# APRIL-ZJU/Ctrl-VIO

Hardware: NVIDIA H100
Metric: residual+Jacobian block evaluations per second (sliding-window LM solve) (higher is better)
Workload: dtype f64

## Files before the change

### ctrl-vio_b200/csrc/engine.cu

```cuda
#include <atomic>
#include <cmath>
#include <cstdlib>
#include <map>

#include "engine_state.h"
#include "poly_min.h"

namespace {

int refresh_mirror(ctvio_engine* e, cudaStream_t on = nullptr) {
  const size_t need = 4 * size_t(e->nK) + kPStride * size_t(e->nK) + 6 * size_t(std::max(e->nB, 1)) + size_t(std::max(e->nL, 1)) + 8;
  if (need > e->h_mirror_cap) {
    if (e->h_mirror) cudaFreeHost(e->h_mirror);
    e->h_mirror = nullptr;
    e->h_mirror_cap = 0;
    if (cudaHostAlloc(reinterpret_cast<void**>(&e->h_mirror), (2 * need) * sizeof(double), cudaHostAllocDefault) != cudaSuccess) {
      cudaGetLastError();
      e->mirror_valid = false;
      return CTVIO_OK;
    }
    e->h_mirror_cap = 2 * need;
  }
  DevState& x = e->x[e->cur];
  double* m = e->h_mirror;
// ... 53 lines not shown
      if (c.t != t) { c.t = t; c.ok = knot_window(e, t, c.f, c.l); }
      f = c.f; l = c.l;
      return c.ok;
    };
    for (int k = 0; k < n; ++k) {
      const HostImage& o = e->img[k];
      int f0, l0, f1, l1;
      if (!window_of(o.ti, f0, l0) || !window_of(o.tj, f1, l1))
        return fail(CTVIO_ERR_TIME_RANGE, "image factor time (+ rolling-shutter padding) outside the spline");
      if (o.lm < 0 || o.lm >= e->nL) return fail(CTVIO_ERR_INVALID, "landmark index out of range");
      wi0[k] = f0; wj0[k] = f1;
      e->img_li[k] = l0; e->img_lj[k] = l1;
      e->h_lo[o.lm] = std::min(e->h_lo[o.lm], 6 * std::min(f0, f1));
      e->h_hi[o.lm] = std::max(e->h_hi[o.lm], 6 * (std::max(l0, l1) + 1));
    }
    e->img_order.resize(n);
    {
      bool lm_sorted = true;
      for (int k = 1; k < n && lm_sorted; ++k) lm_sorted = e->img[k - 1].lm <= e->img[k].lm;
      const size_t nKk = size_t(e->nK) + 1;
      if (lm_sorted && nKk * nKk <= (size_t(1) << 22)) {
        std::vector<int32_t> start(nKk * nKk + 1, 0);
        for (int k = 0; k < n; ++k) ++start[size_t(wi0[k]) * nKk + size_t(wj0[k]) + 1];
        for (size_t g = 1; g < start.size(); ++g) start[g] += start[g - 1];
        for (int k = 0; k < n; ++k) e->img_order[start[size_t(wi0[k]) * nKk + size_t(wj0[k])]++] = k;
      } else {
        std::vector<uint64_t> key(n);
        const uint64_t nLl = uint64_t(std::max(e->nL, 1));
        if (uint64_t(nKk) * nKk * nLl < (uint64_t(1) << 40) && uint64_t(n) < (uint64_t(1) << 24)) {
          for (int k = 0; k < n; ++k)
            key[k] = (((uint64_t(wi0[k]) * nKk + uint64_t(wj0[k])) * nLl + uint64_t(e->img[k].lm)) << 24) | uint64_t(k);
          std::sort(key.begin(), key.end());
          for (int k = 0; k < n; ++k) e->img_order[k] = int32_t(key[k] & 0xffffffu);
        } else {
          for (int k = 0; k < n; ++k) e->img_order[k] = k;
          std::stable_sort(e->img_order.begin(), e->img_order.end(), [&](int a, int b) {
            if (wi0[a] != wi0[b]) return wi0[a] < wi0[b];
            if (wj0[a] != wj0[b]) return wj0[a] < wj0[b];
            return e->img[a].lm < e->img[b].lm;
          });
        }
      }
    }
    std::vector<longlong2> ht(n);
    std::vector<double2> hpi(n), hpj(n);
    std::vector<int4> hm(n);
    for (int k = 0; k < n; ++k) {
      const HostImage& o = e->img[e->img_order[k]];
      ht[k] = make_longlong2(o.ti, o.tj);
      hpi[k] = make_double2(o.pi[0], o.pi[1]);
      hpj[k] = make_double2(o.pj[0], o.pj[1]);
      hm[k] = make_int4(o.rowi, o.rowj, o.lm, o.marg);
    }
    constexpr int cap = kVisObsPerRound;
    std::vector<VisualItem>& items = e->h_items;
    items.clear();
    for (int k = 0; k < n;) {
      const int a = e->img_order[k];
      int end = k;
      while (end < n && wi0[e->img_order[end]] == wi0[a] && wj0[e->img_order[end]] == wj0[a]) ++end;
      const int cnt = end - k;
      const int nchunks = (cnt + cap - 1) / cap;
      const int per = (cnt + nchunks - 1) / nchunks;
      for (int s = k; s < end; s += per) items.push_back(VisualItem{s, std::min(per, end - s), wi0[a], wj0[a]});
      k = end;
    }
    e->n_items = int(items.size());
    if (!e->img_desc.empty()) {
      std::vector<ctvio::FactorDesc> sd(n);
      for (int k = 0; k < n; ++k) sd[k] = e->img_desc[e->img_order[k]];
      CUDA_OK(e->d_img_desc.upload(sd, st));
      CUDA_OK(e->d_img_t.reserve(n)); CUDA_OK(e->d_img_pi.reserve(n)); CUDA_OK(e->d_img_pj.reserve(n)); CUDA_OK(e->d_img_meta.reserve(n));
      ctvio::GatherFactorsArgs ga;
      ga.n = n; ga.desc = e->d_img_desc.p; ga.table = e->d_frames.p; ga.frame_t = e->d_frame_t.p;
      ga.frame_cap = ctvio_engine::kFrameCap;
      ga.t = e->d_img_t.p; ga.pi = e->d_img_pi.p; ga.pj = e->d_img_pj.p; ga.meta = e->d_img_meta.p;
      e->launches += ctvio::launch_gather_factors(ga, st);
    } else {
      CUDA_OK(e->d_img_t.upload(ht, st));
      CUDA_OK(e->d_img_pi.upload(hpi, st));
      CUDA_OK(e->d_img_pj.upload(hpj, st));
      CUDA_OK(e->d_img_meta.upload(hm, st));
    }
    CUDA_OK(e->d_img_orig.upload(e->img_order, st));
    CUDA_OK(e->d_items.upload(items, st));

    e->h_woff.assign(e->nL + 1, 0);
    for (int l = 0; l < e->nL; ++l) {
      if (e->h_hi[l] == 0) e->h_lo[l] = 0;
      e->h_woff[l + 1] = e->h_woff[l] + (e->h_hi[l] - e->h_lo[l]);
    }
    CUDA_OK(e->d_lo.upload(e->h_lo, st));
    CUDA_OK(e->d_hi.upload(e->h_hi, st));
    CUDA_OK(e->d_woff.upload(e->h_woff, st));
    const int ni = int(e->imu.size());
    std::vector<longlong2> it(ni);
    std::vector<double2> iga(3 * size_t(ni));
    const int64_t maxt = e->cfg.t0_ns + int64_t(e->nK - 3) * e->cfg.dt_ns;
    std::vector<int32_t>& imu_order = e->imu_order;
    imu_order.assign(ni, 0);
    std::vector<int32_t> imu_s(ni);
    for (int k = 0; k < ni; ++k) {
      const HostImu& o = e->imu[k];
      if (o.t < e->cfg.t0_ns || o.t >= maxt) return fail(CTVIO_ERR_TIME_RANGE, "imu time outside the spline");
      if (o.node < 0 || o.node >= e->nB) return fail(CTVIO_ERR_INVALID, "bias node out of range");
      imu_order[k] = k;
      imu_s[k] = knot_window_first(e, o.t);
    }
    std::stable_sort(imu_order.begin(), imu_order.end(), [&](int a, int b) {
      if (imu_s[a] != imu_s[b]) return imu_s[a] < imu_s[b];
      return e->imu[a].node < e->imu[b].node;
    });
    std::vector<ImuItem> imu_items;
    for (int k = 0; k < ni; ++k) {
      const HostImu& o = e->imu[imu_order[k]];
      it[k] = make_longlong2(o.t, o.node);
      iga[3 * k] = make_double2(o.gyro[0], o.gyro[1]);
      iga[3 * k + 1] = make_double2(o.gyro[2], o.accel[0]);
// ... 1727 lines not shown
```

### ctrl-vio_b200/csrc/kernels.h

```cpp
#pragma once
#include <cuda_runtime.h>

#include <atomic>

#include <cstdint>
#include <utility>

#include "spline_eval.cuh"

namespace ctvio {

constexpr int kPStride = 4;
constexpr int kVisThreads = 256;
constexpr int kVisObsPerRound = 128;
constexpr int kLocalDim = 64;
constexpr int kRowStride = 66;
constexpr int kObsStride = 2 * kRowStride + 2;
constexpr int kWinKnots = 5;
constexpr int kColLd = 60, kColR = 61, kColRho = 62;
constexpr int kCholNB = 64;

struct StatePtrs {
  double* q;
  double* p;
  double* bias;
  double* rho;
  double* ld;
  KnotPair* tab;
};

struct NormalEqPtrs {
  double* A;
  double* gc;
  double* hl;
  double* gl;
  double* wld;
  double* W;
  double* cost;
};

struct ImageObsPtrs {
  const longlong2* t;
  const double2* pi;
  const double2* pj;
  const int4* meta;
  int32_t n;
};

struct VisualItem {
  int32_t start, count;
  int32_t wi0, wj0;
};

struct ImuObsPtrs {
  const longlong2* t_node;
  const double2* ga;
  int32_t n;
};

struct ImuItem {
  int32_t start, count;
  int32_t s, node;
};
constexpr int kImuMaxPerItem = 32;

struct BiasFactorPtrs {
  const int2* ij;
// ... 263 lines not shown
```

### ctrl-vio_b200/csrc/kernels_residual.cu

```cuda
#include <cstdio>

#include "kernels.h"

namespace ctvio {


__device__ __forceinline__ uint32_t smem_u32(const void* p) { return static_cast<uint32_t>(__cvta_generic_to_shared(p)); }

__device__ __forceinline__ void mbar_init(uint64_t* bar, uint32_t count) {
  asm volatile("mbarrier.init.shared::cta.b64 [%0], %1;" ::"r"(smem_u32(bar)), "r"(count) : "memory");
}
__device__ __forceinline__ void fence_mbar_init() { asm volatile("fence.mbarrier_init.release.cluster;" ::: "memory"); }
__device__ __forceinline__ void mbar_expect_tx(uint64_t* bar, uint32_t bytes) {
  asm volatile("mbarrier.arrive.expect_tx.shared::cta.b64 _, [%0], %1;" ::"r"(smem_u32(bar)), "r"(bytes) : "memory");
}
__device__ __forceinline__ void tma_bulk_g2s(void* dst, const void* src, uint32_t bytes, uint64_t* bar) {
  asm volatile("cp.async.bulk.shared::cluster.global.mbarrier::complete_tx::bytes [%0], [%1], %2, [%3];" ::"r"(
                   smem_u32(dst)),
               "l"(src), "r"(bytes), "r"(smem_u32(bar))
               : "memory");
}
__device__ __forceinline__ bool mbar_try_wait(uint64_t* bar, uint32_t phase) {
  uint32_t ok;
  asm volatile(
// ... 11 lines not shown
__device__ __forceinline__ double warp_sum(double v) {
#pragma unroll
  for (int o = 16; o > 0; o >>= 1) v += __shfl_xor_sync(0xffffffffu, v, o);
  return v;
}


__global__ void knot_table_kernel(StatePtrs st, int nK) {
  const int k = blockIdx.x * blockDim.x + threadIdx.x;
  if (k >= nK - 1) return;
  KnotPair kp;
  make_knot_pair(st.q, k, kp);
  st.tab[k] = kp;
}

int launch_knot_table(const StatePtrs& st, int nK, cudaStream_t s) {
  if (nK < 2) return 0;
  knot_table_kernel<<<(nK - 1 + 127) / 128, 128, 0, s>>>(st, nK);
  return 1;
}


struct VisArgs {
  ImageObsPtrs obs;
  const VisualItem* items;
  StatePtrs st;
  NormalEqPtrs ne;
  LandmarkLayout lm;
  ProblemDims dims;
  SplineParams sp;
  RigParams rig;
  double cauchy;
  const uint8_t* cmask;
  LmScalars* scal;
  int* det_ticket;
};

struct __align__(128) VisStatic {
  KnotPair tab[2][4];
  double q[2][kWinKnots][4];
  double p[2][kWinKnots][4];
  double cost_part[8];
  unsigned long long bar;
  int err;
};

__constant__ uint8_t c_tile_i[36] = {0, 0, 0, 0, 0, 0, 0, 0, 1, 1, 1, 1, 1, 1, 1, 2, 2, 2,
                                     2, 2, 2, 3, 3, 3, 3, 3, 4, 4, 4, 4, 5, 5, 5, 6, 6, 7};
__constant__ uint8_t c_tile_j[36] = {0, 1, 2, 3, 4, 5, 6, 7, 1, 2, 3, 4, 5, 6, 7, 2, 3, 4,
                                     5, 6, 7, 3, 4, 5, 6, 7, 4, 5, 6, 7, 5, 6, 7, 6, 7, 7};

#ifdef CTVIO_CHOL_TIMING
__device__ long long g_vis_clk[8];
#define VCLK(i) do { if (blockIdx.x == 0 && threadIdx.x == 0) g_vis_clk[(i)] = clock64(); } while (0)
extern "C" int ctvio_debug_vis_clk(long long* out) {
  return cudaMemcpyFromSymbol(out, g_vis_clk, sizeof(g_vis_clk)) == cudaSuccess ? 0 : -1;
}
#else
#define VCLK(i)
#endif

size_t visual_smem_bytes() {
  return size_t(kVisObsPerRound) * kObsStride * sizeof(double) + size_t(36) * 64 * sizeof(double);
}

__device__ __noinline__ void syrk_round(const double* Jt, double* accs, int nround, int tid) {
  const int warp = tid >> 5, lane = tid & 31, g = lane >> 2, q = lane & 3;
  const int nblk = warp < 6 ? 1 : 2;
  int bi[2], bj[2];
  if (warp < 6) {
    bi[0] = warp < 3 ? 0 : (warp < 5 ? 1 : 2);
    bj[0] = warp < 3 ? warp + 1 : (warp < 5 ? warp - 1 : 3);
    bi[1] = bj[1] = 0;
  } else {
    bi[0] = bj[0] = 2 * (warp - 6);
    bi[1] = bj[1] = 2 * (warp - 6) + 1;
  }
  const bool dg = warp >= 6;
  double acc[2][2][2][2];
#pragma unroll
  for (int b = 0; b < 2; ++b)
#pragma unroll
    for (int mi = 0; mi < 2; ++mi)
#pragma unroll
      for (int nj = 0; nj < 2; ++nj) {
        const int ti = 2 * bi[b] + mi, tj = 2 * bj[b] + nj;
        double2 v = make_double2(0.0, 0.0);
        if (b < nblk && ti <= tj) v = *reinterpret_cast<const double2*>(accs + (ti * 8 - ti * (ti - 1) / 2 + (tj - ti)) * 64 + g * 8 + 2 * q);
        acc[b][mi][nj][0] = v.x; acc[b][mi][nj][1] = v.y;
      }
  const int nsteps = (2 * nround + 3) >> 2;
#pragma unroll 2
  for (int st = 0; st < nsteps; ++st) {
    const int row = 4 * st + q;
    const double* rp = Jt + size_t(row >> 1) * kObsStride + (row & 1) * kRowStride + g;
#pragma unroll
    for (int b = 0; b < 2; ++b) {
      if (b < nblk) {
        double av[2], bv[2];
#pragma unroll
        for (int m = 0; m < 2; ++m) {
          av[m] = rp[16 * bi[b] + 8 * m];
          bv[m] = dg ? av[m] : rp[16 * bj[b] + 8 * m];
        }
#pragma unroll
        for (int mi = 0; mi < 2; ++mi)
#pragma unroll
          for (int nj = 0; nj < 2; ++nj) {
            if (dg && mi == 1 && nj == 0) continue;
            asm volatile("mma.sync.aligned.m8n8k4.row.col.f64.f64.f64.f64 {%0,%1}, {%2}, {%3}, {%0,%1};"
                         : "+d"(acc[b][mi][nj][0]), "+d"(acc[b][mi][nj][1])
                         : "d"(av[mi]), "d"(bv[nj]));
          }
      }
    }
  }
#pragma unroll
  for (int b = 0; b < 2; ++b)
#pragma unroll
    for (int mi = 0; mi < 2; ++mi)
#pragma unroll
      for (int nj = 0; nj < 2; ++nj) {
        const int ti = 2 * bi[b] + mi, tj = 2 * bj[b] + nj;
        if (b < nblk && ti <= tj)
          *reinterpret_cast<double2*>(accs + (ti * 8 - ti * (ti - 1) / 2 + (tj - ti)) * 64 + g * 8 + 2 * q) =
              make_double2(acc[b][mi][nj][0], acc[b][mi][nj][1]);
      }
  __syncthreads();
}

template <bool FULL>
__global__ void __launch_bounds__(kVisThreads, 1) visual_kernel(const __grid_constant__ VisArgs a) {
  extern __shared__ __align__(128) unsigned char dyn_smem[];
  double* Jt = reinterpret_cast<double*>(dyn_smem);
  double* accs = Jt + size_t(kVisObsPerRound) * kObsStride;
  __shared__ VisStatic sm;

  const int tid = threadIdx.x;
  const int lane = tid & 31, warp = tid >> 5;
  const VisualItem item = a.items[blockIdx.x];
  const int nK = a.dims.nK;
  VCLK(0);

  const int w0[2] = {item.wi0, item.wj0};
  if (tid == 0) {
    sm.err = 0;
    mbar_init(reinterpret_cast<uint64_t*>(&sm.bar), 1);
    fence_mbar_init();
  }
  __syncthreads();
  if (tid == 0) {
    uint32_t bytes = 0;
#pragma unroll
    for (int sd = 0; sd < 2; ++sd) {
      const int nk = min(kWinKnots, nK - w0[sd]);
      const int npair = min(4, nK - 1 - w0[sd]);
      bytes += uint32_t(nk) * 64u + uint32_t(npair) * uint32_t(sizeof(KnotPair));
    }
    mbar_expect_tx(reinterpret_cast<uint64_t*>(&sm.bar), bytes);
#pragma unroll
    for (int sd = 0; sd < 2; ++sd) {
      const int nk = min(kWinKnots, nK - w0[sd]);
      const int npair = min(4, nK - 1 - w0[sd]);
      tma_bulk_g2s(&sm.q[sd][0][0], a.st.q + 4 * w0[sd], uint32_t(nk) * 32u, reinterpret_cast<uint64_t*>(&sm.bar));
      tma_bulk_g2s(&sm.p[sd][0][0], a.st.p + 4 * w0[sd], uint32_t(nk) * 32u, reinterpret_cast<uint64_t*>(&sm.bar));
      tma_bulk_g2s(&sm.tab[sd][0], a.st.tab + w0[sd], uint32_t(npair) * uint32_t(sizeof(KnotPair)),
                   reinterpret_cast<uint64_t*>(&sm.bar));
    }
  }
  if (FULL)
    for (int i = tid; i < 36 * 64; i += kVisThreads) accs[i] = 0.0;
  while (!mbar_try_wait(reinterpret_cast<uint64_t*>(&sm.bar), 0)) {
  }
  __syncthreads();

  const double ld = *a.st.ld;
  const int64_t ld_ns = int64_t(ld * 1e9);
  const int side = tid & 1;
  double cost_local = 0.0;
  VCLK(1);
// ... 180 lines not shown
        const int gb = sb == 0 ? 6 * item.wi0 + lb : (sb == 1 ? 6 * item.wj0 + (lb - 30) : a.dims.idx_ld);
        if (n_class > 1) {
          int c;
          if (sb == 2) c = 5 + sa;
          else if (sa == sb) c = sa == 0 ? 0 : 4;
          else c = ga < gb ? 1 : (ga > gb ? 2 : 3);
          if (c != cls) continue;
        }
        const double v = (la != lb && ga == gb) ? 2.0 * val : val;
        const int g0 = min(ga, gb), g1 = max(ga, gb);
        atomicAdd(a.ne.A + size_t(g0) * np + g1, v);
      }
      if (n_class > 1) {
        __threadfence();
        __syncthreads();
      }
    }
  }
  if (a.det_ticket) {
    __threadfence();
    __syncthreads();
    if (tid == 0) asm volatile("st.release.gpu.global.s32 [%0], %1;" ::"l"(a.det_ticket), "r"((int(blockIdx.x) + 1) * 1024) : "memory");
  }
  VCLK(5);
}

int launch_visual(const VisualLaunch& l, bool full, cudaStream_t s) {
  if (l.n_items <= 0) return 0;
  VisArgs a{l.obs, l.items, l.st, l.ne, l.lm, l.dims, l.sp, l.rig, l.cauchy, l.cmask, l.scal, l.det_ticket};
  static PerDeviceOnce once;
  if (once.first()) {
    cudaFuncSetAttribute(visual_kernel<true>, cudaFuncAttributeMaxDynamicSharedMemorySize, int(visual_smem_bytes()));
    cudaFuncSetAttribute(visual_kernel<false>, cudaFuncAttributeMaxDynamicSharedMemorySize, int(visual_smem_bytes()));
  }
  if (full) visual_kernel<true><<<l.n_items, kVisThreads, visual_smem_bytes(), s>>>(a);
  else visual_kernel<false><<<l.n_items, kVisThreads, 0, s>>>(a);
  return 1;
}


struct ImuArgs {
  ImuObsPtrs obs;
  const ImuItem* items;
  StatePtrs st;
  NormalEqPtrs ne;
  ProblemDims dims;
  SplineParams sp;
  RigParams rig;
  const uint8_t* cmask;
  LmScalars* scal;
  int* det_ticket;
};

constexpr int kImuThreads = 64;
constexpr int kImuCols = 32;
constexpr int kImuRowStride = 34;
__constant__ uint8_t c_imu_tile_i[10] = {0, 0, 0, 0, 1, 1, 1, 2, 2, 3};
__constant__ uint8_t c_imu_tile_j[10] = {0, 1, 2, 3, 1, 2, 3, 2, 3, 3};

template <bool FULL>
__global__ void __launch_bounds__(kImuThreads) imu_kernel(const __grid_constant__ ImuArgs a) {
  extern __shared__ __align__(16) unsigned char dyn_smem[];
  double* Js = reinterpret_cast<double*>(dyn_smem);
  double* accs = Js + kImuMaxPerItem * 6 * kImuRowStride;
  const int tid = threadIdx.x;
  const ImuItem item = a.items[blockIdx.x];
  double cost = 0.0;
  if (FULL)
    for (int i = tid; i < 10 * 64; i += kImuThreads) accs[i] = 0.0;
  if (tid < item.count) {
    const int n = item.start + tid;
    const longlong2 tn = a.obs.t_node[n];
    const double2 g0 = a.obs.ga[3 * n], g1 = a.obs.ga[3 * n + 1], g2 = a.obs.ga[3 * n + 2];
    const double gyro[3] = {g0.x, g0.y, g1.x}, accel[3] = {g1.y, g2.x, g2.y};
    const int node = item.node;
    double bias[6];
#pragma unroll
    for (int c = 0; c < 6; ++c) bias[c] = a.st.bias[6 * node + c];
    int32_t s;
    double u;
    const bool ok = spline_index(a.sp, tn.x, s, u) && s == item.s;
    double* J = Js + size_t(tid) * 6 * kImuRowStride;
    if (!ok) {
      atomicOr(&a.scal->error_flags, 1);
      if (FULL)
        for (int e = 0; e < 6 * kImuRowStride; ++e) J[e] = 0.0;
    } else {
      ImuEvalOut o;
      eval_imu<FULL, kPStride>(a.sp, a.rig, a.st.q, a.st.p, a.st.tab, s, u, gyro, accel, bias, o);
      cost = o.cost;
      if (FULL) {
        const int gb0 = a.dims.idx_bias0 + 6 * node;
#pragma unroll
        for (int r = 0; r < 6; ++r) {
          double* Jr = J + r * kImuRowStride;
#pragma unroll
          for (int k = 0; k < 4; ++k)
#pragma unroll
            for (int c = 0; c < 3; ++c) {
              Jr[k * 6 + c] = a.cmask[6 * (s + k) + c] ? 0.0 : o.Jrot[k][3 * r + c];
              Jr[k * 6 + 3 + c] = a.cmask[6 * (s + k) + 3 + c] ? 0.0 : o.Jpos[k][3 * r + c];
            }
#pragma unroll
          for (int c = 0; c < 6; ++c) Jr[24 + c] = (c == r && !a.cmask[gb0 + c]) ? a.rig.imu_info[r] : 0.0;
          Jr[30] = o.r[r];
          Jr[31] = 0.0;
        }
      }
    }
  }
  if (FULL) {
    __syncthreads();
    const int grp = tid / 10, tile = tid % 10;
    double acc[64];
    if (tid < 60) {
      const int ti = c_imu_tile_i[tile], tj = c_imu_tile_j[tile];
#pragma unroll
      for (int e = 0; e < 64; ++e) acc[e] = 0.0;
      const int nrows = 6 * item.count;
      for (int row = grp; row < nrows; row += 6) {
        const double2* ra = reinterpret_cast<const double2*>(Js + size_t(row) * kImuRowStride + ti * 8);
        const double2* rb = reinterpret_cast<const double2*>(Js + size_t(row) * kImuRowStride + tj * 8);
        double av[8], bv[8];
#pragma unroll
        for (int e = 0; e < 4; ++e) {
          const double2 x = ra[e], y = rb[e];
          av[2 * e] = x.x; av[2 * e + 1] = x.y;
          bv[2 * e] = y.x; bv[2 * e + 1] = y.y;
        }
#pragma unroll
        for (int i = 0; i < 8; ++i)
#pragma unroll
          for (int j = 0; j < 8; ++j) acc[i * 8 + j] = fma(av[i], bv[j], acc[i * 8 + j]);
      }
    }
    for (int g = 0; g < 6; ++g) {
      if (tid < 60 && grp == g) {
#pragma unroll
        for (int e = 0; e < 64; ++e) accs[tile * 64 + e] += acc[e];
      }
      __syncthreads();
    }
    const int np = a.dims.np;
    det_ticket_wait(a.det_ticket, blockIdx.x);
    for (int idx = tid; idx < 10 * 64; idx += kImuThreads) {
      const double val = accs[idx];
      if (val == 0.0) continue;
      const int tile2 = idx >> 6, e = idx & 63;
      const int la = c_imu_tile_i[tile2] * 8 + (e >> 3), lb = c_imu_tile_j[tile2] * 8 + (e & 7);
      if (la > lb || lb > 30 || la >= 30) continue;
      const int ga = la < 24 ? 6 * item.s + la : a.dims.idx_bias0 + 6 * item.node + (la - 24);
      if (lb == 30) {
        atomicAdd(a.ne.gc + ga, val);
        continue;
      }
      const int gb = lb < 24 ? 6 * item.s + lb : a.dims.idx_bias0 + 6 * item.node + (lb - 24);
      atomicAdd(a.ne.A + size_t(ga) * np + gb, val);
    }
  }
  if (!FULL) det_ticket_wait(a.det_ticket, blockIdx.x);
  cost = warp_sum(cost);
  if (tid == 0 && cost != 0.0) atomicAdd(a.ne.cost, cost);
  det_ticket_done(a.det_ticket, blockIdx.x);
}

int launch_imu(const ImuLaunch& l, bool full, cudaStream_t s) {
  if (l.n_items <= 0) return 0;
  ImuArgs a{l.obs, l.items, l.st, l.ne, l.dims, l.sp, l.rig, l.cmask, l.scal, l.det_ticket};
  const size_t smem = (size_t(kImuMaxPerItem) * 6 * kImuRowStride + 10 * 64) * sizeof(double);
  static PerDeviceOnce once;
  if (once.first()) cudaFuncSetAttribute(imu_kernel<true>, cudaFuncAttributeMaxDynamicSharedMemorySize, int(smem));
  if (full) imu_kernel<true><<<l.n_items, kImuThreads, smem, s>>>(a);
  else imu_kernel<false><<<l.n_items, kImuThreads, 0, s>>>(a);
  return 1;
}


struct SmallArgs {
  BiasFactorPtrs bf;
  PriorPtrs prior;
  StatePtrs st;
  NormalEqPtrs ne;
  ProblemDims dims;
  const uint8_t* cmask;
  LmScalars* scal;
  int deterministic;
};

__device__ __forceinline__ const double* block_data(const StatePtrs& st, int type, int index) {
  switch (type) {
    case 0: return st.q + 4 * index;
    case 1: return st.p + kPStride * index;
    case 2: return st.bias + 6 * index;
    case 3: return st.bias + 6 * index + 3;
    case 4: return st.ld;
    default: return st.rho + index;
  }
}

template <bool FULL>
__global__ void __launch_bounds__(256) small_factors_kernel(const __grid_constant__ SmallArgs a) {
  __shared__ double red[8];
  const int tid = threadIdx.x;
  double cost = 0.0;
  const int np = a.dims.np;
  for (int n = a.deterministic ? (tid == 0 ? 0 : a.bf.n) : tid; n < a.bf.n; n += a.deterministic ? 1 : blockDim.x) {
    const int2 ij = a.bf.ij[n];
#pragma unroll
    for (int k = 0; k < 6; ++k) {
      const double s = a.bf.sqrt_info[6 * n + k];
      const double r = s * (a.st.bias[6 * ij.y + k] - a.st.bias[6 * ij.x + k]);
      cost += 0.5 * r * r;
      if (FULL) {
        const int gi = a.dims.idx_bias0 + 6 * ij.x + k, gj = a.dims.idx_bias0 + 6 * ij.y + k;
        const double ji = a.cmask[gi] ? 0.0 : -s, jj = a.cmask[gj] ? 0.0 : s;
        atomicAdd(a.ne.gc + gi, ji * r);
        atomicAdd(a.ne.gc + gj, jj * r);
        atomicAdd(a.ne.A + size_t(gi) * np + gi, ji * ji);
        atomicAdd(a.ne.A + size_t(gj) * np + gj, jj * jj);
        atomicAdd(a.ne.A + size_t(min(gi, gj)) * np + max(gi, gj), ji * jj);
      }
    }
// ... 207 lines not shown
```

### ctrl-vio_b200/csrc/spline_eval.cuh

```cuda
#pragma once
#include "device_math.cuh"

namespace ctvio {

struct KnotPair {
  double d[3];
  double theta;
  double jrinv[9];
  double pad[3];
};

struct SplineParams {
  int64_t t0_ns, dt_ns;
  int32_t n_knots;
  double inv_dt;
};

CTVIO_HD bool spline_index(const SplineParams& sp, int64_t t, int32_t& s, double& u) {
  const int64_t st = t - sp.t0_ns;
  if (st < 0 || t >= sp.t0_ns + int64_t(sp.n_knots - 3) * sp.dt_ns) return false;
  const int64_t si = st / sp.dt_ns;
  s = int32_t(si);
  u = double(st - si * sp.dt_ns) / double(sp.dt_ns);
  return true;
// ... 284 lines not shown
  M3 jv;
#pragma unroll
  for (int e = 0; e < 6; ++e) jv.m[e] = cm.JvR[e];
  jv.m[6] = jv.m[7] = jv.m[8] = 0.0;
  if (side == 0) {
    const M3 t = m3_mul_hat(m3_mul(jv, R_me), cm.p_Ii);
#pragma unroll
    for (int e = 0; e < 6; ++e) lhs[e] = -t.m[e];
  } else {
    const M3 t = m3_mul(m3_mul_hat(jv, cm.dp), R_me);
#pragma unroll
    for (int e = 0; e < 6; ++e) lhs[e] = t.m[e];
  }
}
CTVIO_HD void image_side_blocks(int side, const ImageCommon& cm, const SideEval& me, double rot[4][6], double pos[4][6]) {
  double lhs[6];
  image_side_lhs(side, cm, me.R, lhs);
  const double sgn = side == 0 ? 1.0 : -1.0;
#pragma unroll
  for (int k = 0; k < 4; ++k) {
    mul23_33(lhs, me.J[k], rot[k]);
#pragma unroll
    for (int e = 0; e < 6; ++e) pos[k][e] = sgn * me.c[k] * cm.JvR[e];
  }
}

CTVIO_HD void image_jrho(const RigParams& rig, const ImageCommon& cm, const M3& R_i, double rho, double out[2]) {
  const V3 t = m3_vec(R_i, m3_vec(rig.R_CI, cm.xci));
  const V3 v = V3{-t.x / rho, -t.y / rho, -t.z / rho};
  out[0] = cm.JvR[0] * v.x + cm.JvR[1] * v.y + cm.JvR[2] * v.z;
  out[1] = cm.JvR[3] * v.x + cm.JvR[4] * v.y + cm.JvR[5] * v.z;
}

CTVIO_HD void image_jld(const RigParams& rig, const ImageCommon& cm, int rowi, int rowj, const M3& R_i, V3 om_i, V3 v_i,
                        const M3& R_j, V3 om_j, V3 v_j, double out[2]) {
  const double ri = double(rowi), rj = double(rowj);
  V3 Jx = m3_tvec(R_j, ri * v_i - rj * v_j);
  const V3 a = m3_tvec(R_j, cm.dp);
  Jx = Jx - rj * cross(om_j, a);
  Jx = Jx + ri * m3_tvec(R_j, m3_vec(R_i, cross(om_i, cm.p_Ii)));
  const V3 y = m3_tvec(rig.R_CI, Jx);
  out[0] = cm.Jv[0] * y.x + cm.Jv[1] * y.y + cm.Jv[2] * y.z;
  out[1] = cm.Jv[3] * y.x + cm.Jv[4] * y.y + cm.Jv[5] * y.z;
}

struct ImuEvalOut {
  int32_t s;
  double r[6];
  double Jrot[4][18];
  double Jpos[4][18];
  double cost;
};

template <bool WANT_JAC, int PS>
CTVIO_HD void eval_imu(const SplineParams& sp, const RigParams& rig, const double* q, const double* p,
                       const KnotPair* tab, int32_t s, double u, const double gyro[3], const double accel[3],
                       const double bias[6], ImuEvalOut& o) {
  o.s = s;
  double lam[4], dl[4], ca[4];
  cum_coeffs(u, lam);
  cum_dcoeffs(u, sp.inv_dt, dl);
  plain_coeffs<2>(u, sp.inv_dt, ca);
  V3 acc = ca[0] * load_p<PS>(p, s);
#pragma unroll
  for (int k = 1; k < 4; ++k) acc = acc + ca[k] * load_p<PS>(p, s + k);
  Q4 E[3];
  V3 phi[3], d[3];
#pragma unroll
  for (int j = 0; j < 3; ++j) {
    const KnotPair& kp = tab[s + j];
    d[j] = V3{kp.d[0], kp.d[1], kp.d[2]};
    phi[j] = lam[j + 1] * d[j];
    const double th = fabs(lam[j + 1]) * kp.theta;
    E[j] = so3_exp_theta(neg(phi[j]), th * th, th);
  }
  const Q4 B3 = E[2];
  const Q4 B32 = so3_mul(B3, E[1]);
  const Q4 B321 = so3_mul(B32, E[0]);
  V3 om[4];
  om[0] = V3{0, 0, 0};
#pragma unroll
  for (int i = 0; i < 3; ++i) om[i + 1] = so3_rotate(E[i], om[i]) + dl[i + 1] * d[i];
  const Q4 Rinv_q = so3_mul(B321, q_conj(load_q(q, s)));
  const M3 Rinv = so3_matrix(Rinv_q);
  const V3 ag = acc + rig.gravity;
  const V3 a_body = so3_rotate(Rinv_q, ag);
  const V3 g = om[3];
  o.r[0] = rig.imu_info[0] * (g.x - (gyro[0] - bias[0]));
  o.r[1] = rig.imu_info[1] * (g.y - (gyro[1] - bias[1]));
  o.r[2] = rig.imu_info[2] * (g.z - (gyro[2] - bias[2]));
  o.r[3] = rig.imu_info[3] * (a_body.x - (accel[0] - bias[3]));
  o.r[4] = rig.imu_info[4] * (a_body.y - (accel[1] - bias[4]));
  o.r[5] = rig.imu_info[5] * (a_body.z - (accel[2] - bias[5]));
  double cs = 0;
#pragma unroll
  for (int k = 0; k < 6; ++k) cs += o.r[k] * o.r[k];
  o.cost = 0.5 * cs;
  if (!WANT_JAC) return;

  const M3 P[4] = {so3_matrix(B321), so3_matrix(B32), so3_matrix(B3), m3_identity()};
  M3 JrN[3], JI[3];
#pragma unroll
  for (int j = 0; j < 3; ++j) {
    JrN[j] = right_jacobian_from_half(neg(phi[j]), E[j]);
#pragma unroll
    for (int e = 0; e < 9; ++e) JI[j].m[e] = tab[s + j].jrinv[e];
  }
  M3 dw[3];
  dw[0] = m3_scale(dl[1], P[1]);
#pragma unroll
  for (int i = 1; i < 3; ++i) {
    const M3 t = m3_mul(m3_mul_hat(P[i], om[i]), JrN[i]);
#pragma unroll
    for (int e = 0; e < 9; ++e) dw[i].m[e] = lam[i + 1] * t.m[e] + dl[i + 1] * P[i + 1].m[e];
  }
  M3 Jw[4], Ja[4];
#pragma unroll
  for (int k = 0; k < 4; ++k)
#pragma unroll
    for (int e = 0; e < 9; ++e) Jw[k].m[e] = Ja[k].m[e] = 0.0;
#pragma unroll
  for (int i = 0; i < 3; ++i) {
    const M3 a = m3_mul_bt(dw[i], JI[i]), b = m3_mul(dw[i], JI[i]);
#pragma unroll
    for (int e = 0; e < 9; ++e) { Jw[i].m[e] -= a.m[e]; Jw[i + 1].m[e] += b.m[e]; }
  }
  const M3 R = m3_transpose(Rinv);
  const M3 lhs = m3_mul_hat(Rinv, ag);
  const M3 lR = m3_mul(lhs, R);
  {
    const M3 t = m3_mul(lR, P[0]);
#pragma unroll
    for (int e = 0; e < 9; ++e) Ja[0].m[e] += t.m[e];
  }
#pragma unroll
  for (int i = 0; i < 3; ++i) {
    const M3 da = m3_scale(lam[i + 1], m3_mul(m3_mul(lR, P[i]), JrN[i]));
    const M3 a = m3_mul_bt(da, JI[i]), b = m3_mul(da, JI[i]);
#pragma unroll
    for (int e = 0; e < 9; ++e) { Ja[i].m[e] -= a.m[e]; Ja[i + 1].m[e] += b.m[e]; }
  }
#pragma unroll
  for (int k = 0; k < 4; ++k)
#pragma unroll
    for (int r = 0; r < 3; ++r)
#pragma unroll
      for (int c = 0; c < 3; ++c) {
        o.Jrot[k][3 * r + c] = rig.imu_info[r] * Jw[k].m[3 * r + c];
        o.Jrot[k][9 + 3 * r + c] = rig.imu_info[3 + r] * Ja[k].m[3 * r + c];
        o.Jpos[k][3 * r + c] = 0.0;
        o.Jpos[k][9 + 3 * r + c] = rig.imu_info[3 + r] * (ca[k] * Rinv.m[3 * r + c]);
      }
}

}
```

Before: 33.05 million.

## Split IMU Jacobian across warps with FP64 MMA syrk and adaptive visual chunking

The IMU kernel moves from 64 threads with scalar FMA outer products to 128 threads. Each of four warps computes one quarter of the Jacobian (gyro or accel rows, first or second knot pair) into a column-major shared tile, then accumulates its assigned 8x8 tiles with FP64 mma.sync and flushes them straight to global memory via atomics. Visual work items are split into smaller chunks, down to a minimum of 64, when the resulting count still fits within the SM count. The visual syrk is also templated so that diagonal and off-diagonal warps compile separately. The IMU stage computation is now duplicated in every warp, trading that redundant work for parallelism and removing the shared-memory reduction loop.

New measurement: 34.77 million, median of 6. +5.2%, better.

```diff
diff --git a/ctrl-vio_b200/csrc/engine.cu b/ctrl-vio_b200/csrc/engine.cu
--- a/ctrl-vio_b200/csrc/engine.cu
+++ b/ctrl-vio_b200/csrc/engine.cu
@@ -129,18 +129,30 @@
       hpj[k] = make_double2(o.pj[0], o.pj[1]);
       hm[k] = make_int4(o.rowi, o.rowj, o.lm, o.marg);
     }
-    constexpr int cap = kVisObsPerRound;
-    std::vector<VisualItem>& items = e->h_items;
-    items.clear();
+    std::vector<int2> groups;
     for (int k = 0; k < n;) {
       const int a = e->img_order[k];
       int end = k;
       while (end < n && wi0[e->img_order[end]] == wi0[a] && wj0[e->img_order[end]] == wj0[a]) ++end;
-      const int cnt = end - k;
+      groups.push_back(make_int2(k, end));
+      k = end;
+    }
+    auto n_chunks = [&](int c) {
+      size_t m = 0;
+      for (const int2& g : groups) m += (g.y - g.x + c - 1) / c;
+      return m;
+    };
+    int cap = kVisObsPerRound;
+    const size_t n_sm = size_t(device_sm_count());
+    while (cap / 2 >= kVisMinChunk && n_chunks(cap / 2) <= n_sm) cap /= 2;
+    std::vector<VisualItem>& items = e->h_items;
+    items.clear();
+    for (const int2& g : groups) {
+      const int a = e->img_order[g.x];
+      const int cnt = g.y - g.x;
       const int nchunks = (cnt + cap - 1) / cap;
       const int per = (cnt + nchunks - 1) / nchunks;
-      for (int s = k; s < end; s += per) items.push_back(VisualItem{s, std::min(per, end - s), wi0[a], wj0[a]});
-      k = end;
+      for (int s = g.x; s < g.y; s += per) items.push_back(VisualItem{s, std::min(per, g.y - s), wi0[a], wj0[a]});
     }
     e->n_items = int(items.size());
     if (!e->img_desc.empty()) {
diff --git a/ctrl-vio_b200/csrc/kernels.h b/ctrl-vio_b200/csrc/kernels.h
--- a/ctrl-vio_b200/csrc/kernels.h
+++ b/ctrl-vio_b200/csrc/kernels.h
@@ -13,6 +13,7 @@
 constexpr int kPStride = 4;
 constexpr int kVisThreads = 256;
 constexpr int kVisObsPerRound = 128;
+constexpr int kVisMinChunk = 64;
 constexpr int kLocalDim = 64;
 constexpr int kRowStride = 66;
 constexpr int kObsStride = 2 * kRowStride + 2;
diff --git a/ctrl-vio_b200/csrc/kernels_residual.cu b/ctrl-vio_b200/csrc/kernels_residual.cu
--- a/ctrl-vio_b200/csrc/kernels_residual.cu
+++ b/ctrl-vio_b200/csrc/kernels_residual.cu
@@ -87,41 +87,46 @@
 
 #ifdef CTVIO_CHOL_TIMING
 __device__ long long g_vis_clk[8];
+__device__ long long g_imu_clk[8];
 #define VCLK(i) do { if (blockIdx.x == 0 && threadIdx.x == 0) g_vis_clk[(i)] = clock64(); } while (0)
+#define ICLK(i) do { if (blockIdx.x == 0 && threadIdx.x == 0) g_imu_clk[(i)] = clock64(); } while (0)
 extern "C" int ctvio_debug_vis_clk(long long* out) {
   return cudaMemcpyFromSymbol(out, g_vis_clk, sizeof(g_vis_clk)) == cudaSuccess ? 0 : -1;
 }
+extern "C" int ctvio_debug_imu_clk(long long* out) {
+  return cudaMemcpyFromSymbol(out, g_imu_clk, sizeof(g_imu_clk)) == cudaSuccess ? 0 : -1;
+}
 #else
 #define VCLK(i)
+#define ICLK(i)
 #endif
 
 size_t visual_smem_bytes() {
   return size_t(kVisObsPerRound) * kObsStride * sizeof(double) + size_t(36) * 64 * sizeof(double);
 }
 
-__device__ __noinline__ void syrk_round(const double* Jt, double* accs, int nround, int tid) {
-  const int warp = tid >> 5, lane = tid & 31, g = lane >> 2, q = lane & 3;
-  const int nblk = warp < 6 ? 1 : 2;
-  int bi[2], bj[2];
-  if (warp < 6) {
+template <bool DIAG>
+__device__ __noinline__ void syrk_round_warp(const double* Jt, double* accs, int nround, int warp, int lane) {
+  constexpr int NB = DIAG ? 2 : 1;
+  const int g = lane >> 2, q = lane & 3;
+  int bi[NB], bj[NB];
+  if constexpr (DIAG) {
+    bi[0] = bj[0] = 2 * (warp - 6);
+    bi[1] = bj[1] = 2 * (warp - 6) + 1;
+  } else {
     bi[0] = warp < 3 ? 0 : (warp < 5 ? 1 : 2);
     bj[0] = warp < 3 ? warp + 1 : (warp < 5 ? warp - 1 : 3);
-    bi[1] = bj[1] = 0;
-  } else {
-    bi[0] = bj[0] = 2 * (warp - 6);
-    bi[1] = bj[1] = 2 * (warp - 6) + 1;
-  }
-  const bool dg = warp >= 6;
-  double acc[2][2][2][2];
-#pragma unroll
-  for (int b = 0; b < 2; ++b)
+  }
+  double acc[NB][2][2][2];
+#pragma unroll
+  for (int b = 0; b < NB; ++b)
 #pragma unroll
     for (int mi = 0; mi < 2; ++mi)
 #pragma unroll
       for (int nj = 0; nj < 2; ++nj) {
+        if (DIAG && mi == 1 && nj == 0) continue;
         const int ti = 2 * bi[b] + mi, tj = 2 * bj[b] + nj;
-        double2 v = make_double2(0.0, 0.0);
-        if (b < nblk && ti <= tj) v = *reinterpret_cast<const double2*>(accs + (ti * 8 - ti * (ti - 1) / 2 + (tj - ti)) * 64 + g * 8 + 2 * q);
+        const double2 v = *reinterpret_cast<const double2*>(accs + (ti * 8 - ti * (ti - 1) / 2 + (tj - ti)) * 64 + g * 8 + 2 * q);
         acc[b][mi][nj][0] = v.x; acc[b][mi][nj][1] = v.y;
       }
   const int nsteps = (2 * nround + 3) >> 2;
@@ -130,37 +135,41 @@
     const int row = 4 * st + q;
     const double* rp = Jt + size_t(row >> 1) * kObsStride + (row & 1) * kRowStride + g;
 #pragma unroll
-    for (int b = 0; b < 2; ++b) {
-      if (b < nblk) {
-        double av[2], bv[2];
-#pragma unroll
-        for (int m = 0; m < 2; ++m) {
-          av[m] = rp[16 * bi[b] + 8 * m];
-          bv[m] = dg ? av[m] : rp[16 * bj[b] + 8 * m];
+    for (int b = 0; b < NB; ++b) {
+      double av[2], bv[2];
+#pragma unroll
+      for (int m = 0; m < 2; ++m) {
+        av[m] = rp[16 * bi[b] + 8 * m];
+        bv[m] = DIAG ? av[m] : rp[16 * bj[b] + 8 * m];
+      }
+#pragma unroll
+      for (int mi = 0; mi < 2; ++mi)
+#pragma unroll
+        for (int nj = 0; nj < 2; ++nj) {
+          if (DIAG && mi == 1 && nj == 0) continue;
+          asm volatile("mma.sync.aligned.m8n8k4.row.col.f64.f64.f64.f64 {%0,%1}, {%2}, {%3}, {%0,%1};"
+                       : "+d"(acc[b][mi][nj][0]), "+d"(acc[b][mi][nj][1])
+                       : "d"(av[mi]), "d"(bv[nj]));
         }
-#pragma unroll
-        for (int mi = 0; mi < 2; ++mi)
-#pragma unroll
-          for (int nj = 0; nj < 2; ++nj) {
-            if (dg && mi == 1 && nj == 0) continue;
-            asm volatile("mma.sync.aligned.m8n8k4.row.col.f64.f64.f64.f64 {%0,%1}, {%2}, {%3}, {%0,%1};"
-                         : "+d"(acc[b][mi][nj][0]), "+d"(acc[b][mi][nj][1])
-                         : "d"(av[mi]), "d"(bv[nj]));
-          }
-      }
-    }
-  }
-#pragma unroll
-  for (int b = 0; b < 2; ++b)
+    }
+  }
+#pragma unroll
+  for (int b = 0; b < NB; ++b)
 #pragma unroll
     for (int mi = 0; mi < 2; ++mi)
 #pragma unroll
       for (int nj = 0; nj < 2; ++nj) {
+        if (DIAG && mi == 1 && nj == 0) continue;
         const int ti = 2 * bi[b] + mi, tj = 2 * bj[b] + nj;
-        if (b < nblk && ti <= tj)
-          *reinterpret_cast<double2*>(accs + (ti * 8 - ti * (ti - 1) / 2 + (tj - ti)) * 64 + g * 8 + 2 * q) =
-              make_double2(acc[b][mi][nj][0], acc[b][mi][nj][1]);
-      }
+        *reinterpret_cast<double2*>(accs + (ti * 8 - ti * (ti - 1) / 2 + (tj - ti)) * 64 + g * 8 + 2 * q) =
+            make_double2(acc[b][mi][nj][0], acc[b][mi][nj][1]);
+      }
+}
+
+__device__ __forceinline__ void syrk_round(const double* Jt, double* accs, int nround, int tid) {
+  const int warp = tid >> 5, lane = tid & 31;
+  if (warp < 6) syrk_round_warp<false>(Jt, accs, nround, warp, lane);
+  else syrk_round_warp<true>(Jt, accs, nround, warp, lane);
   __syncthreads();
 }
 
@@ -447,24 +456,109 @@
   int* det_ticket;
 };
 
-constexpr int kImuThreads = 64;
+constexpr int kImuThreads = 128;
 constexpr int kImuCols = 32;
-constexpr int kImuRowStride = 34;
-__constant__ uint8_t c_imu_tile_i[10] = {0, 0, 0, 0, 1, 1, 1, 2, 2, 3};
-__constant__ uint8_t c_imu_tile_j[10] = {0, 1, 2, 3, 1, 2, 3, 2, 3, 3};
+constexpr int kImuColStride = 196;
+static_assert(kImuColStride >= 6 * kImuMaxPerItem && kImuColStride % 16 == 4, "K2 shared column stride");
+
+__host__ __device__ constexpr int imu_tile(int w, int t) {
+  return w == 0 ? (t == 0 ? 0 : t == 1 ? 1 : 5)
+       : w == 1 ? (t == 0 ? 10 : t == 1 ? 11 : 15)
+       : w == 2 ? (t == 0 ? 2 : 3)
+                : (t == 0 ? 6 : 7);
+}
+__host__ __device__ constexpr int imu_ntiles(int w) { return w < 2 ? 3 : 2; }
+__host__ __device__ constexpr bool imu_uses(int w, int c) {
+  bool u = false;
+  for (int t = 0; t < imu_ntiles(w); ++t) u = u || imu_tile(w, t) >> 2 == c || (imu_tile(w, t) & 3) == c;
+  return u;
+}
+
+__device__ __forceinline__ void imu_zero_part(double* J, int warp) {
+  const int r0 = 3 * (warp >> 1), c0 = 12 * (warp & 1), c1 = (warp & 1) ? kImuCols : 12;
+  for (int c = c0; c < c1; ++c)
+#pragma unroll
+    for (int r = 0; r < 3; ++r) J[c * kImuColStride + r0 + r] = 0.0;
+}
+
+template <bool ACCEL, int H>
+__device__ __forceinline__ void imu_write_part(const ImuArgs& a, const ImuStage& st, int s, int node, double* J) {
+  constexpr int r0 = ACCEL ? 3 : 0;
+  imu_jacobian_half<ACCEL, H>(a.rig, a.st.tab, s, st, [&](int k, const double rot[9], const double pos[9]) {
+#pragma unroll
+    for (int c = 0; c < 3; ++c) {
+      const bool mr = a.cmask[6 * (s + k) + c] != 0, mp = a.cmask[6 * (s + k) + 3 + c] != 0;
+#pragma unroll
+      for (int r = 0; r < 3; ++r) {
+        J[(k * 6 + c) * kImuColStride + r0 + r] = mr ? 0.0 : rot[3 * r + c];
+        J[(k * 6 + 3 + c) * kImuColStride + r0 + r] = mp ? 0.0 : pos[3 * r + c];
+      }
+    }
+  });
+  if (H == 1) {
+    const int gb0 = a.dims.idx_bias0 + 6 * node;
+#pragma unroll
+    for (int c = 0; c < 6; ++c) {
+      const bool mb = a.cmask[gb0 + c] != 0;
+#pragma unroll
+      for (int r = 0; r < 3; ++r) J[(24 + c) * kImuColStride + r0 + r] = (c == r0 + r && !mb) ? a.rig.imu_info[r0 + r] : 0.0;
+    }
+#pragma unroll
+    for (int r = 0; r < 3; ++r) {
+      J[30 * kImuColStride + r0 + r] = st.r[r0 + r];
+      J[31 * kImuColStride + r0 + r] = 0.0;
+    }
+  }
+}
+
+template <int W>
+__device__ __forceinline__ void imu_syrk(const double* Js, int nsteps, int lane, double acc[3][2]) {
+  const double* rp = Js + (lane >> 2) * kImuColStride + (lane & 3);
+#pragma unroll
+  for (int t = 0; t < 3; ++t) acc[t][0] = acc[t][1] = 0.0;
+#pragma unroll 4
+  for (int st = 0; st < nsteps; ++st, rp += 4) {
+    double v[4];
+#pragma unroll
+    for (int c = 0; c < 4; ++c) v[c] = imu_uses(W, c) ? rp[8 * c * kImuColStride] : 0.0;
+#pragma unroll
+    for (int t = 0; t < imu_ntiles(W); ++t)
+      asm volatile("mma.sync.aligned.m8n8k4.row.col.f64.f64.f64.f64 {%0,%1}, {%2}, {%3}, {%0,%1};"
+                   : "+d"(acc[t][0]), "+d"(acc[t][1])
+                   : "d"(v[imu_tile(W, t) >> 2]), "d"(v[imu_tile(W, t) & 3]));
+  }
+}
+
+template <int W>
+__device__ __forceinline__ void imu_flush(const ImuArgs& a, const ImuItem& item, int lane, const double acc[3][2]) {
+  const int np = a.dims.np;
+#pragma unroll
+  for (int t = 0; t < imu_ntiles(W); ++t)
+#pragma unroll
+    for (int e = 0; e < 2; ++e) {
+      const double val = acc[t][e];
+      const int la = 8 * (imu_tile(W, t) >> 2) + (lane >> 2), lb = 8 * (imu_tile(W, t) & 3) + 2 * (lane & 3) + e;
+      if (val == 0.0 || la > lb || lb > 30 || la >= 30) continue;
+      const int ga = la < 24 ? 6 * item.s + la : a.dims.idx_bias0 + 6 * item.node + (la - 24);
+      if (lb == 30) {
+        atomicAdd(a.ne.gc + ga, val);
+        continue;
+      }
+      const int gb = lb < 24 ? 6 * item.s + lb : a.dims.idx_bias0 + 6 * item.node + (lb - 24);
+      atomicAdd(a.ne.A + size_t(ga) * np + gb, val);
+    }
+}
 
 template <bool FULL>
 __global__ void __launch_bounds__(kImuThreads) imu_kernel(const __grid_constant__ ImuArgs a) {
-  extern __shared__ __align__(16) unsigned char dyn_smem[];
+  extern __shared__ __align__(128) unsigned char dyn_smem[];
   double* Js = reinterpret_cast<double*>(dyn_smem);
-  double* accs = Js + kImuMaxPerItem * 6 * kImuRowStride;
-  const int tid = threadIdx.x;
+  const int tid = threadIdx.x, warp = tid >> 5, lane = tid & 31;
   const ImuItem item = a.items[blockIdx.x];
   double cost = 0.0;
-  if (FULL)
-    for (int i = tid; i < 10 * 64; i += kImuThreads) accs[i] = 0.0;
-  if (tid < item.count) {
-    const int n = item.start + tid;
+  ICLK(0);
+  if ((FULL || warp == 0) && lane < item.count) {
+    const int n = item.start + lane;
     const longlong2 tn = a.obs.t_node[n];
     const double2 g0 = a.obs.ga[3 * n], g1 = a.obs.ga[3 * n + 1], g2 = a.obs.ga[3 * n + 2];
     const double gyro[3] = {g0.x, g0.y, g1.x}, accel[3] = {g1.y, g2.x, g2.y};
@@ -475,94 +569,61 @@
     int32_t s;
     double u;
     const bool ok = spline_index(a.sp, tn.x, s, u) && s == item.s;
-    double* J = Js + size_t(tid) * 6 * kImuRowStride;
+    double* J = Js + 6 * lane;
     if (!ok) {
-      atomicOr(&a.scal->error_flags, 1);
-      if (FULL)
-        for (int e = 0; e < 6 * kImuRowStride; ++e) J[e] = 0.0;
+      if (warp == 0) atomicOr(&a.scal->error_flags, 1);
+      if (FULL) imu_zero_part(J, warp);
     } else {
-      ImuEvalOut o;
-      eval_imu<FULL, kPStride>(a.sp, a.rig, a.st.q, a.st.p, a.st.tab, s, u, gyro, accel, bias, o);
-      cost = o.cost;
+      ImuStage st;
+      imu_stage<kPStride>(a.sp, a.rig, a.st.q, a.st.p, a.st.tab, s, u, gyro, accel, bias, st);
+      cost = st.cost;
       if (FULL) {
-        const int gb0 = a.dims.idx_bias0 + 6 * node;
-#pragma unroll
-        for (int r = 0; r < 6; ++r) {
-          double* Jr = J + r * kImuRowStride;
-#pragma unroll
-          for (int k = 0; k < 4; ++k)
-#pragma unroll
-            for (int c = 0; c < 3; ++c) {
-              Jr[k * 6 + c] = a.cmask[6 * (s + k) + c] ? 0.0 : o.Jrot[k][3 * r + c];
-              Jr[k * 6 + 3 + c] = a.cmask[6 * (s + k) + 3 + c] ? 0.0 : o.Jpos[k][3 * r + c];
-            }
-#pragma unroll
-          for (int c = 0; c < 6; ++c) Jr[24 + c] = (c == r && !a.cmask[gb0 + c]) ? a.rig.imu_info[r] : 0.0;
-          Jr[30] = o.r[r];
-          Jr[31] = 0.0;
+        switch (warp) {
+          case 0: imu_write_part<false, 0>(a, st, s, node, J); break;
+          case 1: imu_write_part<false, 1>(a, st, s, node, J); break;
+          case 2: imu_write_part<true, 0>(a, st, s, node, J); break;
+          default: imu_write_part<true, 1>(a, st, s, node, J); break;
         }
       }
     }
+  } else if (FULL && lane == item.count) {
+    imu_zero_part(Js + 6 * lane, warp);
   }
   if (FULL) {
+    ICLK(1);
     __syncthreads();
-    const int grp = tid / 10, tile = tid % 10;
-    double acc[64];
-    if (tid < 60) {
-      const int ti = c_imu_tile_i[tile], tj = c_imu_tile_j[tile];
-#pragma unroll
-      for (int e = 0; e < 64; ++e) acc[e] = 0.0;
-      const int nrows = 6 * item.count;
-      for (int row = grp; row < nrows; row += 6) {
-        const double2* ra = reinterpret_cast<const double2*>(Js + size_t(row) * kImuRowStride + ti * 8);
-        const double2* rb = reinterpret_cast<const double2*>(Js + size_t(row) * kImuRowStride + tj * 8);
-        double av[8], bv[8];
-#pragma unroll
-        for (int e = 0; e < 4; ++e) {
-          const double2 x = ra[e], y = rb[e];
-          av[2 * e] = x.x; av[2 * e + 1] = x.y;
-          bv[2 * e] = y.x; bv[2 * e + 1] = y.y;
-        }
-#pragma unroll
-        for (int i = 0; i < 8; ++i)
-#pragma unroll
-          for (int j = 0; j < 8; ++j) acc[i * 8 + j] = fma(av[i], bv[j], acc[i * 8 + j]);
-      }
-    }
-    for (int g = 0; g < 6; ++g) {
-      if (tid < 60 && grp == g) {
-#pragma unroll
-        for (int e = 0; e < 64; ++e) accs[tile * 64 + e] += acc[e];
-      }
-      __syncthreads();
-    }
-    const int np = a.dims.np;
+    ICLK(2);
+    const int nsteps = (6 * item.count + 3) >> 2;
+    double acc[3][2];
+    switch (warp) {
+      case 0: imu_syrk<0>(Js, nsteps, lane, acc); break;
+      case 1: imu_syrk<1>(Js, nsteps, lane, acc); break;
+      case 2: imu_syrk<2>(Js, nsteps, lane, acc); break;
+      default: imu_syrk<3>(Js, nsteps, lane, acc); break;
+    }
+    ICLK(3);
+    ICLK(4);
     det_ticket_wait(a.det_ticket, blockIdx.x);
-    for (int idx = tid; idx < 10 * 64; idx += kImuThreads) {
-      const double val = accs[idx];
-      if (val == 0.0) continue;
-      const int tile2 = idx >> 6, e = idx & 63;
-      const int la = c_imu_tile_i[tile2] * 8 + (e >> 3), lb = c_imu_tile_j[tile2] * 8 + (e & 7);
-      if (la > lb || lb > 30 || la >= 30) continue;
-      const int ga = la < 24 ? 6 * item.s + la : a.dims.idx_bias0 + 6 * item.node + (la - 24);
-      if (lb == 30) {
-        atomicAdd(a.ne.gc + ga, val);
-        continue;
-      }
-      const int gb = lb < 24 ? 6 * item.s + lb : a.dims.idx_bias0 + 6 * item.node + (lb - 24);
-      atomicAdd(a.ne.A + size_t(ga) * np + gb, val);
-    }
+    switch (warp) {
+      case 0: imu_flush<0>(a, item, lane, acc); break;
+      case 1: imu_flush<1>(a, item, lane, acc); break;
+      case 2: imu_flush<2>(a, item, lane, acc); break;
+      default: imu_flush<3>(a, item, lane, acc); break;
+    }
+    ICLK(5);
   }
   if (!FULL) det_ticket_wait(a.det_ticket, blockIdx.x);
-  cost = warp_sum(cost);
-  if (tid == 0 && cost != 0.0) atomicAdd(a.ne.cost, cost);
+  if (warp == 0) {
+    cost = warp_sum(cost);
+    if (lane == 0 && cost != 0.0) atomicAdd(a.ne.cost, cost);
+  }
   det_ticket_done(a.det_ticket, blockIdx.x);
 }
 
 int launch_imu(const ImuLaunch& l, bool full, cudaStream_t s) {
   if (l.n_items <= 0) return 0;
   ImuArgs a{l.obs, l.items, l.st, l.ne, l.dims, l.sp, l.rig, l.cmask, l.scal, l.det_ticket};
-  const size_t smem = (size_t(kImuMaxPerItem) * 6 * kImuRowStride + 10 * 64) * sizeof(double);
+  const size_t smem = size_t(kImuCols) * kImuColStride * sizeof(double);
   static PerDeviceOnce once;
   if (once.first()) cudaFuncSetAttribute(imu_kernel<true>, cudaFuncAttributeMaxDynamicSharedMemorySize, int(smem));
   if (full) imu_kernel<true><<<l.n_items, kImuThreads, smem, s>>>(a);
diff --git a/ctrl-vio_b200/csrc/spline_eval.cuh b/ctrl-vio_b200/csrc/spline_eval.cuh
--- a/ctrl-vio_b200/csrc/spline_eval.cuh
+++ b/ctrl-vio_b200/csrc/spline_eval.cuh
@@ -360,40 +360,44 @@
   double cost;
 };
 
-template <bool WANT_JAC, int PS>
-CTVIO_HD void eval_imu(const SplineParams& sp, const RigParams& rig, const double* q, const double* p,
-                       const KnotPair* tab, int32_t s, double u, const double gyro[3], const double accel[3],
-                       const double bias[6], ImuEvalOut& o) {
-  o.s = s;
+struct ImuStage {
   double lam[4], dl[4], ca[4];
-  cum_coeffs(u, lam);
-  cum_dcoeffs(u, sp.inv_dt, dl);
-  plain_coeffs<2>(u, sp.inv_dt, ca);
-  V3 acc = ca[0] * load_p<PS>(p, s);
-#pragma unroll
-  for (int k = 1; k < 4; ++k) acc = acc + ca[k] * load_p<PS>(p, s + k);
-  Q4 E[3];
-  V3 phi[3], d[3];
+  V3 phi[3];
+  Q4 E[3], B32, B321;
+  V3 om[4];
+  Q4 Rinv_q;
+  V3 ag;
+  double r[6], cost;
+};
+
+template <int PS>
+CTVIO_HD void imu_stage(const SplineParams& sp, const RigParams& rig, const double* q, const double* p,
+                        const KnotPair* tab, int32_t s, double u, const double gyro[3], const double accel[3],
+                        const double bias[6], ImuStage& o) {
+  cum_coeffs(u, o.lam);
+  cum_dcoeffs(u, sp.inv_dt, o.dl);
+  plain_coeffs<2>(u, sp.inv_dt, o.ca);
+  V3 acc = o.ca[0] * load_p<PS>(p, s);
+#pragma unroll
+  for (int k = 1; k < 4; ++k) acc = acc + o.ca[k] * load_p<PS>(p, s + k);
+  V3 d[3];
 #pragma unroll
   for (int j = 0; j < 3; ++j) {
     const KnotPair& kp = tab[s + j];
     d[j] = V3{kp.d[0], kp.d[1], kp.d[2]};
-    phi[j] = lam[j + 1] * d[j];
-    const double th = fabs(lam[j + 1]) * kp.theta;
-    E[j] = so3_exp_theta(neg(phi[j]), th * th, th);
-  }
-  const Q4 B3 = E[2];
-  const Q4 B32 = so3_mul(B3, E[1]);
-  const Q4 B321 = so3_mul(B32, E[0]);
-  V3 om[4];
-  om[0] = V3{0, 0, 0};
-#pragma unroll
-  for (int i = 0; i < 3; ++i) om[i + 1] = so3_rotate(E[i], om[i]) + dl[i + 1] * d[i];
-  const Q4 Rinv_q = so3_mul(B321, q_conj(load_q(q, s)));
-  const M3 Rinv = so3_matrix(Rinv_q);
-  const V3 ag = acc + rig.gravity;
-  const V3 a_body = so3_rotate(Rinv_q, ag);
-  const V3 g = om[3];
+    o.phi[j] = o.lam[j + 1] * d[j];
+    const double th = fabs(o.lam[j + 1]) * kp.theta;
+    o.E[j] = so3_exp_theta(neg(o.phi[j]), th * th, th);
+  }
+  o.B32 = so3_mul(o.E[2], o.E[1]);
+  o.B321 = so3_mul(o.B32, o.E[0]);
+  o.om[0] = V3{0, 0, 0};
+#pragma unroll
+  for (int i = 0; i < 3; ++i) o.om[i + 1] = so3_rotate(o.E[i], o.om[i]) + o.dl[i + 1] * d[i];
+  o.Rinv_q = so3_mul(o.B321, q_conj(load_q(q, s)));
+  o.ag = acc + rig.gravity;
+  const V3 a_body = so3_rotate(o.Rinv_q, o.ag);
+  const V3 g = o.om[3];
   o.r[0] = rig.imu_info[0] * (g.x - (gyro[0] - bias[0]));
   o.r[1] = rig.imu_info[1] * (g.y - (gyro[1] - bias[1]));
   o.r[2] = rig.imu_info[2] * (g.z - (gyro[2] - bias[2]));
@@ -404,61 +408,86 @@
 #pragma unroll
   for (int k = 0; k < 6; ++k) cs += o.r[k] * o.r[k];
   o.cost = 0.5 * cs;
+}
+
+template <int I>
+CTVIO_HD M3 imu_P(const ImuStage& st) {
+  if (I == 0) return so3_matrix(st.B321);
+  if (I == 1) return so3_matrix(st.B32);
+  if (I == 2) return so3_matrix(st.E[2]);
+  return m3_identity();
+}
+
+template <bool ACCEL, int I>
+CTVIO_HD M3 imu_dX(const ImuStage& st, const M3& lR) {
+  const M3 JrN = right_jacobian_from_half(neg(st.phi[I]), st.E[I]);
+  if (ACCEL) return m3_scale(st.lam[I + 1], m3_mul(m3_mul(lR, imu_P<I>(st)), JrN));
+  if (I == 0) return m3_scale(st.dl[1], imu_P<1>(st));
+  const M3 t = m3_mul(m3_mul_hat(imu_P<I>(st), st.om[I]), JrN);
+  const M3 Pn = imu_P<I + 1>(st);
+  M3 out;
+#pragma unroll
+  for (int e = 0; e < 9; ++e) out.m[e] = st.lam[I + 1] * t.m[e] + st.dl[I + 1] * Pn.m[e];
+  return out;
+}
+
+template <bool ACCEL, int H, class Emit>
+CTVIO_HD void imu_jacobian_half(const RigParams& rig, const KnotPair* tab, int32_t s, const ImuStage& st, Emit&& emit) {
+  const M3 Rinv = so3_matrix(st.Rinv_q);
+  M3 lR;
+  if (ACCEL) lR = m3_mul(m3_mul_hat(Rinv, st.ag), m3_transpose(Rinv));
+  const M3 Xa = imu_dX<ACCEL, H>(st, lR), Xb = imu_dX<ACCEL, H + 1>(st, lR);
+  M3 JIa, JIb;
+#pragma unroll
+  for (int e = 0; e < 9; ++e) { JIa.m[e] = tab[s + H].jrinv[e]; JIb.m[e] = tab[s + H + 1].jrinv[e]; }
+  M3 J[2];
+  if (H == 0) {
+    const M3 a = m3_mul_bt(Xa, JIa);
+    M3 base;
+    if (ACCEL) base = m3_mul(lR, imu_P<0>(st));
+#pragma unroll
+    for (int e = 0; e < 9; ++e) J[0].m[e] = (ACCEL ? 0.0 + base.m[e] : 0.0) - a.m[e];
+    J[1] = m3_sub(m3_mul(Xa, JIa), m3_mul_bt(Xb, JIb));
+  } else {
+    J[0] = m3_sub(m3_mul(Xa, JIa), m3_mul_bt(Xb, JIb));
+    J[1] = m3_mul(Xb, JIb);
+  }
+#pragma unroll
+  for (int h = 0; h < 2; ++h) {
+    const int k = 2 * H + h;
+    double rot[9], pos[9];
+#pragma unroll
+    for (int r = 0; r < 3; ++r)
+#pragma unroll
+      for (int c = 0; c < 3; ++c) {
+        rot[3 * r + c] = rig.imu_info[(ACCEL ? 3 : 0) + r] * J[h].m[3 * r + c];
+        pos[3 * r + c] = ACCEL ? rig.imu_info[3 + r] * (st.ca[k] * Rinv.m[3 * r + c]) : 0.0;
+      }
+    emit(k, rot, pos);
+  }
+}
+
+template <bool WANT_JAC, int PS>
+CTVIO_HD void eval_imu(const SplineParams& sp, const RigParams& rig, const double* q, const double* p,
+                       const KnotPair* tab, int32_t s, double u, const double gyro[3], const double accel[3],
+                       const double bias[6], ImuEvalOut& o) {
+  ImuStage st;
+  imu_stage<PS>(sp, rig, q, p, tab, s, u, gyro, accel, bias, st);
+  o.s = s;
+#pragma unroll
+  for (int k = 0; k < 6; ++k) o.r[k] = st.r[k];
+  o.cost = st.cost;
   if (!WANT_JAC) return;
-
-  const M3 P[4] = {so3_matrix(B321), so3_matrix(B32), so3_matrix(B3), m3_identity()};
-  M3 JrN[3], JI[3];
-#pragma unroll
-  for (int j = 0; j < 3; ++j) {
-    JrN[j] = right_jacobian_from_half(neg(phi[j]), E[j]);
-#pragma unroll
-    for (int e = 0; e < 9; ++e) JI[j].m[e] = tab[s + j].jrinv[e];
-  }
-  M3 dw[3];
-  dw[0] = m3_scale(dl[1], P[1]);
-#pragma unroll
-  for (int i = 1; i < 3; ++i) {
-    const M3 t = m3_mul(m3_mul_hat(P[i], om[i]), JrN[i]);
-#pragma unroll
-    for (int e = 0; e < 9; ++e) dw[i].m[e] = lam[i + 1] * t.m[e] + dl[i + 1] * P[i + 1].m[e];
-  }
-  M3 Jw[4], Ja[4];
-#pragma unroll
-  for (int k = 0; k < 4; ++k)
-#pragma unroll
-    for (int e = 0; e < 9; ++e) Jw[k].m[e] = Ja[k].m[e] = 0.0;
-#pragma unroll
-  for (int i = 0; i < 3; ++i) {
-    const M3 a = m3_mul_bt(dw[i], JI[i]), b = m3_mul(dw[i], JI[i]);
-#pragma unroll
-    for (int e = 0; e < 9; ++e) { Jw[i].m[e] -= a.m[e]; Jw[i + 1].m[e] += b.m[e]; }
-  }
-  const M3 R = m3_transpose(Rinv);
-  const M3 lhs = m3_mul_hat(Rinv, ag);
-  const M3 lR = m3_mul(lhs, R);
-  {
-    const M3 t = m3_mul(lR, P[0]);
-#pragma unroll
-    for (int e = 0; e < 9; ++e) Ja[0].m[e] += t.m[e];
-  }
-#pragma unroll
-  for (int i = 0; i < 3; ++i) {
-    const M3 da = m3_scale(lam[i + 1], m3_mul(m3_mul(lR, P[i]), JrN[i]));
-    const M3 a = m3_mul_bt(da, JI[i]), b = m3_mul(da, JI[i]);
-#pragma unroll
-    for (int e = 0; e < 9; ++e) { Ja[i].m[e] -= a.m[e]; Ja[i + 1].m[e] += b.m[e]; }
-  }
-#pragma unroll
-  for (int k = 0; k < 4; ++k)
-#pragma unroll
-    for (int r = 0; r < 3; ++r)
-#pragma unroll
-      for (int c = 0; c < 3; ++c) {
-        o.Jrot[k][3 * r + c] = rig.imu_info[r] * Jw[k].m[3 * r + c];
-        o.Jrot[k][9 + 3 * r + c] = rig.imu_info[3 + r] * Ja[k].m[3 * r + c];
-        o.Jpos[k][3 * r + c] = 0.0;
-        o.Jpos[k][9 + 3 * r + c] = rig.imu_info[3 + r] * (ca[k] * Rinv.m[3 * r + c]);
-      }
-}
-
-}
+  auto put = [&o](int row0) {
+    return [&o, row0](int k, const double rot[9], const double pos[9]) {
+#pragma unroll
+      for (int e = 0; e < 9; ++e) { o.Jrot[k][row0 + e] = rot[e]; o.Jpos[k][row0 + e] = pos[e]; }
+    };
+  };
+  imu_jacobian_half<false, 0>(rig, tab, s, st, put(0));
+  imu_jacobian_half<false, 1>(rig, tab, s, st, put(0));
+  imu_jacobian_half<true, 0>(rig, tab, s, st, put(9));
+  imu_jacobian_half<true, 1>(rig, tab, s, st, put(9));
+}
+
+}
```
